# werner-duvaud/muzero-general

Hardware: AMD Instinct MI355X
Metric: mcts_simulations_per_sec (higher is better)
Workload: dtype f32; 1 GPU; C2 CartPole FullyConnectedNetwork, 4096 trees x 50 sims per GPU; trees_per_gpu=4096, num_simulations=50, action_space=2, network=fullyconnected, search_kernel=mzx::fc2_search_kernel, tree_statistics_dtype=f64, weights=reference constructor, torch.manual_seed(0) (RCCL-broadcast flat buffer)

## Files before the change

muzero-general_amd/csrc/mzx_fused_fc.h:

```cpp
#pragma once
#include <stdlib.h>

#include "mzx_search.h"

namespace mzx {

constexpr int FUSED_ROW = 16;
constexpr int FUSED_MAX_WIDTH = 64;
constexpr int FUSED_SCRATCH = 5 * FUSED_MAX_WIDTH;
constexpr int FUSED_PROF_WORDS = 16;

inline int row_action_lanes(const SearchParams& p) {
  const bool wide = p.num_actions > FUSED_ROW || 2 * p.support_size + 1 > 2 * FUSED_ROW;
  return wide ? 0 : (p.num_actions <= 4 ? 4 : 16);
}

struct FusedMlp {
  int32_t n;
  int32_t sizes[MZX_MAX_LAYERS + 2];
  int32_t w[MZX_MAX_LAYERS + 1], b[MZX_MAX_LAYERS + 1];
};

struct FusedFcArgs {
  SearchParams p;
// ... 277 lines not shown
      const int ld = (c == top) ? (depth & (FUSED_ROW - 1)) : FUSED_ROW - 1;
      const bool same = (k.tp == r.c.to_play);
      const double r_eff = (P == 1 || !same) ? k.rr : -k.rr;
      double my_in = val;
      chain_step<FUSED_ROW - 1>(r_eff, p.discount, ld, sub, val, my_in);
      if (sub == 0) my_in = val;
      if (c > 0) val = bcast_d<0>(r_eff) + p.discount * val;
      double qv = 0.0;
      if (k.active) {
        const double vs2 = k.vs + ((P == 1 || same) ? my_in : -my_in);
        const int vc2 = k.vc + 1;
        const double mean = vs2 / (double)vc2;
        qv = k.rr + p.discount * ((P == 1) ? mean : -mean);
        t.value_sum(k.n) = vs2;
        t.visit(k.n) = vc2;
        if (k.par >= 0) { t.slot_visit(k.par, k.ps) = vc2; t.slot_q(k.par, k.ps) = qv; }
        if (k.is_leaf) {
          t.child(k.par, k.ps) = k.n;
          t.parent(k.n) = k.par; t.parent_slot(k.n) = k.ps; t.to_play(k.n) = r.c.to_play; t.reward(k.n) = reward;
        }
      }
      const double h2 = row_max_d<16>(k.active ? qv : -MZX_INF), l2 = row_min_d16(k.active ? qv : MZX_INF);
      hi = h2 > hi ? h2 : hi;
      lo = l2 < lo ? l2 : lo;
      k = up;
    }
    if (hi > st.mx) st.mx = hi;
    if (lo < st.mn) st.mn = lo;
    return;
  }
  if (depth >= FUSED_ROW) {
    if (sub == 0) {
      store_state(t, st);
      t.child(r.c.parent, r.c.slot) = r.c.leaf;
      t.parent(r.c.leaf) = r.c.parent; t.parent_slot(r.c.leaf) = r.c.slot; t.to_play(r.c.leaf) = r.c.to_play;
      t.reward(r.c.leaf) = reward; t.visit(r.c.leaf) = 0; t.value_sum(r.c.leaf) = 0.0;
      tree_backprop(t, p, r.c, value);
    }
    wave_sync();
    st.mn = t.mm_min(); st.mx = t.mm_max();
    return;
  }
  const bool active = sub <= depth, is_leaf = sub == depth;
  const int n = r.my_node;
  double rr = reward, vs = 0.0;
  int vc = 0, tp = r.c.to_play;
  if (active && !is_leaf) {
    rr = t.reward(n); vs = t.value_sum(n); vc = t.visit(n);
    if (P == 2) tp = t.to_play(n);
  }
  const bool same = (tp == r.c.to_play);
  const double r_eff = (P == 1 || !same) ? rr : -rr;
  double val = value, my_in = value;
  chain_step<FUSED_ROW - 1>(r_eff, p.discount, depth, sub, val, my_in);
  if (sub == 0) my_in = val;
  double qv = 0.0;
  if (active) {
    const double vs2 = vs + ((P == 1 || same) ? my_in : -my_in);
    const int vc2 = vc + 1;
    const double mean = vs2 / (double)vc2;
    qv = rr + p.discount * ((P == 1) ? mean : -mean);
    t.value_sum(n) = vs2;
    t.visit(n) = vc2;
    if (sub > 0) { t.slot_visit(r.my_parent, r.my_pslot) = vc2; t.slot_q(r.my_parent, r.my_pslot) = qv; }
    if (is_leaf) {
      t.child(r.my_parent, r.my_pslot) = n;
      t.parent(n) = r.my_parent; t.parent_slot(n) = r.my_pslot; t.to_play(n) = r.c.to_play; t.reward(n) = reward;
    }
  }
  if (row_bits(__ballot(active && (qv > st.mx || qv < st.mn)), row_in_wave)) {
    const double hi = row_max_d<16>(active ? qv : -MZX_INF), lo = row_min_d16(active ? qv : MZX_INF);
    if (hi > st.mx) st.mx = hi;
    if (lo < st.mn) st.mn = lo;
  }
}


struct NetOut { float value, reward, policy; };

struct LdsNet {
  const float* W;
  const FusedFcArgs* a;

  __device__ __forceinline__ void stage_mlp(const FusedMlp& m, const float* flat, float* w, int tid) {
    for (int l = 0; l < m.n; ++l) {
      const int K = m.sizes[l], O = m.sizes[l + 1], base = m.w[l];
      for (int i = tid; i < O * K; i += blockDim.x) {
        const int o = i / K, k = i - o * K;
        w[base + k * O + o] = flat[base + i];
      }
      for (int i = tid; i < O; i += blockDim.x) w[m.b[l] + i] = flat[m.b[l] + i];
    }
  }
  __device__ __forceinline__ void stage(const FusedFcArgs& args, char* smem, int tid) {
    float* w = (float*)(smem + args.lds_weights);
    stage_mlp(args.rep, args.flat, w, tid);
    stage_mlp(args.dyn, args.flat, w, tid);
    stage_mlp(args.rew, args.flat, w, tid);
    stage_mlp(args.pol, args.flat, w, tid);
    stage_mlp(args.val, args.flat, w, tid);
  }
  __device__ __forceinline__ void setup(const FusedFcArgs& args, char* smem, int) {
    W = (const float*)(smem + args.lds_weights);
    a = &args;
  }

  template <int G>
  __device__ __forceinline__ void layer(const float* wl, const float* bl, const float* x, float* y, int K, int Kx, int O,
                                        int sub, int action, bool onehot, bool last) const {
    for (int o0 = sub; o0 < O; o0 += G * FUSED_ROW) {
      const float* wr = wl + o0;
      float acc[G];
#pragma unroll
      for (int j = 0; j < G; ++j) acc[j] = 0.f;
      int k = 0;
      constexpr int U = (G == 1) ? 8 : 4;
      for (; k + U <= Kx; k += U) {
        float xv[U], wv[U][G];
#pragma unroll
        for (int u = 0; u < U; ++u) {
          xv[u] = x[k + u];
#pragma unroll
          for (int j = 0; j < G; ++j) wv[u][j] = wr[(k + u) * O + j * FUSED_ROW];
        }
#pragma unroll
        for (int u = 0; u < U; ++u)
#pragma unroll
          for (int j = 0; j < G; ++j) acc[j] = fmaf(xv[u], wv[u][j], acc[j]);
      }
      for (; k < Kx; ++k) {
        const float xk = x[k];
#pragma unroll
        for (int j = 0; j < G; ++j) acc[j] = fmaf(xk, wr[k * O + j * FUSED_ROW], acc[j]);
      }
#pragma unroll
      for (int j = 0; j < G; ++j) {
        const int o = o0 + j * FUSED_ROW;
        if (o < O) {
          float v = acc[j];
          if (onehot) v += wr[(Kx + action) * O + j * FUSED_ROW];
          v += bl[o];
          y[o] = last ? v : mzx_elu(v);
        }
      }
    }
  }

  __device__ __forceinline__ void mlp(const FusedMlp& m, const float* x, float* tmp0, float* tmp1, float* out, int sub,
                                      int action, int onehot) const {
    for (int l = 0; l < m.n; ++l) {
      const int K = m.sizes[l], O = m.sizes[l + 1];
      const int Kx = (l == 0) ? K - onehot : K;
      const bool last = (l == m.n - 1);
      float* y = last ? out : ((l & 1) ? tmp1 : tmp0);
      const float* wl = W + m.w[l];
      const float* bl = W + m.b[l];
      const bool oh = (l == 0 && onehot);
      if (O > 2 * FUSED_ROW) layer<4>(wl, bl, x, y, K, Kx, O, sub, action, oh, last);
      else if (O > FUSED_ROW) layer<2>(wl, bl, x, y, K, Kx, O, sub, action, oh, last);
      else layer<1>(wl, bl, x, y, K, Kx, O, sub, action, oh, last);
      wave_sync();
      x = y;
    }
  }
  __device__ __forceinline__ void scale(const float* x, float* y, int E, int sub) const {
    float lo = x[0], hi = x[0];
    for (int k = 1; k < E; ++k) { lo = fminf(lo, x[k]); hi = fmaxf(hi, x[k]); }
    float sc = hi - lo;
    if (sc < 1e-5f) sc += 1e-5f;
    for (int j = sub; j < E; j += FUSED_ROW) y[j] = mzx_div(x[j] - lo, sc);
    wave_sync();
  }
  __device__ __forceinline__ float decode(const float* lg, int sub) const {
    const int F = 2 * a->p.support_size + 1, S = a->p.support_size;
    float m = -MZX_INF;
    for (int i = sub; i < F; i += FUSED_ROW) m = fmaxf(m, lg[i]);
    m = row_max(m);
    float den = 0.f;
    for (int i = sub; i < F; i += FUSED_ROW) den += mzx_expf(lg[i] - m);
    den = row_sum(den);
    float num = 0.f;
    for (int i = sub; i < F; i += FUSED_ROW) num += (float)(i - S) * mzx_div(mzx_expf(lg[i] - m), den);
    return support_inverse_transform(row_sum(num));
  }
  __device__ __forceinline__ void heads(const float* h, float* scr, int sub, NetOut& o) const {
    float* s0 = scr; float* s1 = scr + FUSED_MAX_WIDTH; float* s2 = scr + 2 * FUSED_MAX_WIDTH;
    float* s3 = scr + 3 * FUSED_MAX_WIDTH;
// ... 70 lines not shown

__device__ __forceinline__ void dot8x3_bcast(float xs, float xh, const float (&wr)[8], const float (&wp)[8],
                                             const float (&wv)[8], float& r, float& p, float& v) {
  float a = 0.f, b = 0.f, c = 0.f;
#define MZX_STEP3(K, J) MZX_FD_X("%[a]", "%[xs]", "%[r" #J "]", K) MZX_FD_X("%[b]", "%[xh]", "%[p" #J "]", K) MZX_FD_X("%[c]", "%[xh]", "%[v" #J "]", K)
  asm("s_nop 1\n\t" MZX_STEP3(0, 0) MZX_STEP3(1, 1) MZX_STEP3(2, 2) MZX_STEP3(3, 3)
      : [a] "+v"(a), [b] "+v"(b), [c] "+v"(c)
      : [xs] "v"(xs), [xh] "v"(xh), [r0] "v"(wr[0]), [r1] "v"(wr[1]), [r2] "v"(wr[2]), [r3] "v"(wr[3]),
        [p0] "v"(wp[0]), [p1] "v"(wp[1]), [p2] "v"(wp[2]), [p3] "v"(wp[3]),
        [v0] "v"(wv[0]), [v1] "v"(wv[1]), [v2] "v"(wv[2]), [v3] "v"(wv[3]));
  asm("s_nop 1\n\t" MZX_STEP3(4, 0) MZX_STEP3(5, 1) MZX_STEP3(6, 2) MZX_STEP3(7, 3)
      : [a] "+v"(a), [b] "+v"(b), [c] "+v"(c)
      : [xs] "v"(xs), [xh] "v"(xh), [r0] "v"(wr[4]), [r1] "v"(wr[5]), [r2] "v"(wr[6]), [r3] "v"(wr[7]),
        [p0] "v"(wp[4]), [p1] "v"(wp[5]), [p2] "v"(wp[6]), [p3] "v"(wp[7]),
        [v0] "v"(wv[4]), [v1] "v"(wv[5]), [v2] "v"(wv[6]), [v3] "v"(wv[7]));
#undef MZX_STEP3
  r = a; p = b; v = c;
}

__device__ __forceinline__ void dot16x5_bcast(float xr, float xp, float xv, const float (&ra)[16], const float (&rb)[16],
                                              const float (&pw)[16], const float (&va)[16], const float (&vb)[16],
                                              float& o_ra, float& o_rb, float& o_p, float& o_va, float& o_vb) {
  float a = 0.f, b = 0.f, c = 0.f, d = 0.f, e = 0.f;
#define MZX_STEP5(K, J)                                                                                             \
  MZX_FD_X("%[a]", "%[xr]", "%[s" #J "]", K) MZX_FD_X("%[b]", "%[xr]", "%[t" #J "]", K) MZX_FD_X("%[c]", "%[xp]", "%[u" #J "]", K) \
  MZX_FD_X("%[d]", "%[xv]", "%[w" #J "]", K) MZX_FD_X("%[e]", "%[xv]", "%[z" #J "]", K)
#define MZX_BLOCK5(K0, K1, K2, K3, B)                                                                              \
  asm("s_nop 1\n\t" MZX_STEP5(K0, 0) MZX_STEP5(K1, 1) MZX_STEP5(K2, 2) MZX_STEP5(K3, 3)                             \
      : [a] "+v"(a), [b] "+v"(b), [c] "+v"(c), [d] "+v"(d), [e] "+v"(e)                                             \
      : [xr] "v"(xr), [xp] "v"(xp), [xv] "v"(xv),                                                                    \
        [s0] "v"(ra[B]), [s1] "v"(ra[B + 1]), [s2] "v"(ra[B + 2]), [s3] "v"(ra[B + 3]),                               \
        [t0] "v"(rb[B]), [t1] "v"(rb[B + 1]), [t2] "v"(rb[B + 2]), [t3] "v"(rb[B + 3]),                               \
        [u0] "v"(pw[B]), [u1] "v"(pw[B + 1]), [u2] "v"(pw[B + 2]), [u3] "v"(pw[B + 3]),                               \
        [w0] "v"(va[B]), [w1] "v"(va[B + 1]), [w2] "v"(va[B + 2]), [w3] "v"(va[B + 3]),                               \
        [z0] "v"(vb[B]), [z1] "v"(vb[B + 1]), [z2] "v"(vb[B + 2]), [z3] "v"(vb[B + 3]))
  MZX_BLOCK5(0, 1, 2, 3, 0);
  MZX_BLOCK5(4, 5, 6, 7, 4);
  MZX_BLOCK5(8, 9, 10, 11, 8);
  MZX_BLOCK5(12, 13, 14, 15, 12);
#undef MZX_BLOCK5
#undef MZX_STEP5
  o_ra = a; o_rb = b; o_p = c; o_va = d; o_vb = e;
}

__device__ __forceinline__ void row_decode2x2(float a0, float a1, float b0, float b1, int F, int support, int sub,
                                              float& out_a, float& out_b) {
  const bool v0 = sub < F, v1 = sub + 16 < F;
  float ma = fmaxf(v0 ? a0 : -MZX_INF, v1 ? a1 : -MZX_INF), mb = fmaxf(v0 ? b0 : -MZX_INF, v1 ? b1 : -MZX_INF);
  row_max_2(ma, mb);
  const float ea0 = v0 ? mzx_expf(a0 - ma) : 0.f, ea1 = v1 ? mzx_expf(a1 - ma) : 0.f;
  const float eb0 = v0 ? mzx_expf(b0 - mb) : 0.f, eb1 = v1 ? mzx_expf(b1 - mb) : 0.f;
  float da = 0.f, db = 0.f;
  da += ea0; db += eb0;
  if (v1) { da += ea1; db += eb1; }
  const float dena = row_sum(da), denb = row_sum(db);
  float na = 0.f, nb = 0.f;
  if (v0) { na += (float)(sub - support) * mzx_div(ea0, dena); nb += (float)(sub - support) * mzx_div(eb0, denb); }
  if (v1) { na += (float)(sub + 16 - support) * mzx_div(ea1, dena); nb += (float)(sub + 16 - support) * mzx_div(eb1, denb); }
  support_inverse_transform_2(row_sum(na), row_sum(nb), sub, out_a, out_b);
}

template <int K, int I = 0>
__device__ __forceinline__ float fma_bcast(float x, const float (&w)[K], float acc) {
  if constexpr (I < K) {
    acc = fmaf(bcast<I>(x), w[I], acc);
    return fma_bcast<K, I + 1>(x, w, acc);
  } else {
    return acc;
  }
}
template <int K>
__device__ __forceinline__ float dot_bcast(float x, const float (&w)[K]) {
  if constexpr (K == 8) return dot8_bcast(x, w);
  else if constexpr (K == 16) return dot16_bcast(x, w);
  else return fma_bcast<K>(x, w, 0.f);
}
template <int K>
__device__ __forceinline__ void dot2_bcast(float x, const float (&u)[K], const float (&v)[K], float& ru, float& rv) {
  if constexpr (K == 16) dot16x2_bcast(x, u, v, ru, rv);
  else { ru = fma_bcast<K>(x, u, 0.f); rv = fma_bcast<K>(x, v, 0.f); }
}

template <int K>
__device__ __forceinline__ void load_row(float (&w)[K], float& b, const float* flat, int woff, int boff, int o, int O) {
  const bool ok = o < O;
#pragma unroll
  for (int k = 0; k < K; ++k) w[k] = ok ? flat[woff + o * K + k] : 0.f;
  b = ok ? flat[boff + o] : 0.f;
}

template <int IN, int E, int A, int F, int HD, int HR, int HP, int HV>
struct SmallNet {
  static_assert(IN <= 64 && E <= 16 && A <= 16 && F <= 32 && HD <= 16 && HR <= 16 && HP <= 16 && HV <= 16, "shape");
  float w_rep[IN], b_rep;
  float w_d1[E + A], b_d1, w_d2[HD], b_d2;
  float w_r1[E], b_r1, w_r2a[HR], b_r2a, w_r2b[HR], b_r2b;
  float w_p1[E], b_p1, w_p2[HP], b_p2;
  float w_v1[E], b_v1, w_v2a[HV], b_v2a, w_v2b[HV], b_v2b;
  int support;

  static bool matches(const FusedFcArgs& a) {
    const int Fa = 2 * a.p.support_size + 1;
    return a.in_size == IN && a.E == E && a.p.num_actions == A && Fa == F && a.rep.n == 1 && a.dyn.n == 2 &&
           a.dyn.sizes[1] == HD && a.rew.n == 2 && a.rew.sizes[1] == HR && a.pol.n == 2 && a.pol.sizes[1] == HP &&
           a.val.n == 2 && a.val.sizes[1] == HV;
  }

  __device__ __forceinline__ void stage(const FusedFcArgs&, char*, int) {}
  __device__ __forceinline__ void setup(const FusedFcArgs& a, char*, int sub) {
    const float* f = a.flat;
    support = a.p.support_size;
    load_row(w_rep, b_rep, f, a.rep.w[0], a.rep.b[0], sub, E);
    load_row(w_d1, b_d1, f, a.dyn.w[0], a.dyn.b[0], sub, HD);
    load_row(w_d2, b_d2, f, a.dyn.w[1], a.dyn.b[1], sub, E);
    load_row(w_r1, b_r1, f, a.rew.w[0], a.rew.b[0], sub, HR);
    load_row(w_r2a, b_r2a, f, a.rew.w[1], a.rew.b[1], sub, F);
    load_row(w_r2b, b_r2b, f, a.rew.w[1], a.rew.b[1], sub + 16, F);
    load_row(w_p1, b_p1, f, a.pol.w[0], a.pol.b[0], sub, HP);
    load_row(w_p2, b_p2, f, a.pol.w[1], a.pol.b[1], sub, A);
    load_row(w_v1, b_v1, f, a.val.w[0], a.val.b[0], sub, HV);
    load_row(w_v2a, b_v2a, f, a.val.w[1], a.val.b[1], sub, F);
    load_row(w_v2b, b_v2b, f, a.val.w[1], a.val.b[1], sub + 16, F);
  }

  __device__ __forceinline__ float scale(float s, int sub) const {
    const bool in = sub < E;
    float lo = in ? s : MZX_INF, hi = in ? s : -MZX_INF;
    row_min_max(lo, hi);
    float sc = hi - lo;
    if (sc < 1e-5f) sc += 1e-5f;
    return mzx_div(s - lo, sc);
  }
  __device__ __forceinline__ void heads(float hn, int sub, NetOut& o) const {
    const float p1 = mzx_elu(dot_bcast<E>(hn, w_p1) + b_p1);
    const float v1 = mzx_elu(dot_bcast<E>(hn, w_v1) + b_v1);
    o.policy = dot_bcast<HP>(p1, w_p2) + b_p2;
    float va, vb;
    dot2_bcast<HV>(v1, w_v2a, w_v2b, va, vb);
    o.value = row_decode2(va + b_v2a, vb + b_v2b, F, support, sub);
  }
  __device__ __forceinline__ void initial(const float* obs, float* h_out, float*, int sub, NetOut& o) const {
    float acc = 0.f;
#pragma unroll
    for (int k = 0; k < IN; ++k) acc = fmaf(obs[k], w_rep[k], acc);
    const float hn = scale(acc + b_rep, sub);
    h_out[sub] = hn;
    heads(hn, sub, o);
  }
  __device__ __forceinline__ void recurrent(const float* h_in, int action, float* h_out, float*, int sub,
                                            NetOut& o) const {
    float acc = 0.f;
#pragma unroll
    for (int k = 0; k < E; ++k) acc = fmaf(h_in[k], w_d1[k], acc);
    float col = w_d1[E];
#pragma unroll
    for (int x = 1; x < A; ++x) col = (action == x) ? w_d1[E + x] : col;
    const float d1 = mzx_elu((acc + col) + b_d1);
    const float s = dot_bcast<HD>(d1, w_d2) + b_d2;
    if constexpr (E == 8 && HR == 16 && HP == 16 && HV == 16) {
      const float hn = scale(s, sub);
      h_out[sub] = hn;
      float r1, p1, v1;
      dot8x3_bcast(s, hn, w_r1, w_p1, w_v1, r1, p1, v1);
      r1 = mzx_elu(r1 + b_r1); p1 = mzx_elu(p1 + b_p1); v1 = mzx_elu(v1 + b_v1);
      float ra, rb, pl, va, vb;
      dot16x5_bcast(r1, p1, v1, w_r2a, w_r2b, w_p2, w_v2a, w_v2b, ra, rb, pl, va, vb);
      o.policy = pl + b_p2;
      row_decode2x2(va + b_v2a, vb + b_v2b, ra + b_r2a, rb + b_r2b, F, support, sub, o.value, o.reward);
      return;
    }
    const float r1 = mzx_elu(dot_bcast<E>(s, w_r1) + b_r1);
    float ra, rb;
    dot2_bcast<HR>(r1, w_r2a, w_r2b, ra, rb);
    const float hn = scale(s, sub);
    h_out[sub] = hn;
    o.reward = row_decode2(ra + b_r2a, rb + b_r2b, F, support, sub);
    heads(hn, sub, o);
  }
};


#define MZX_PROF(k)                                             \
  if (PROFILE) {                                                \
    __builtin_amdgcn_sched_barrier(0);                          \
    asm volatile("s_waitcnt vmcnt(0) lgkmcnt(0)" ::: "memory"); \
    const unsigned long long _t = __builtin_readcyclecounter(); \
    prof[k] += (uint32_t)(_t - t_last);                         \
    t_last = _t;                                                \
    __builtin_amdgcn_sched_barrier(0);                          \
  }

template <class Net, int AW, bool PROFILE>
__global__ void __launch_bounds__(256) fused_fc_search_kernel(const FusedFcArgs a) {
  extern __shared__ __attribute__((aligned(16))) char smem[];
  const int tid = threadIdx.x;
  const int sub = tid & (FUSED_ROW - 1);
  const int row = tid / FUSED_ROW;
  const int row_in_wave = row & 3;
  const int tree = blockIdx.x * a.trees_per_block + row;
  const int A = a.p.num_actions, E = a.E;
  uint32_t prof[FUSED_PROF_WORDS];
  unsigned long long t_last = 0;
  if (PROFILE) {
    for (int k = 0; k < FUSED_PROF_WORDS; ++k) prof[k] = 0;
    t_last = __builtin_readcyclecounter();
  }

  Net net;
  double* tables = (double*)(smem + a.lds_tables);
  const int ntab = 2 * (a.p.num_nodes + 1);
  for (int i = tid; i < ntab; i += blockDim.x) tables[i] = a.tables[i];
  net.stage(a, smem, tid);
  __syncthreads();
  if (row >= a.trees_per_block || tree >= a.p.num_trees) return;
  net.setup(a, smem, sub);

  char* slab = smem + a.lds_trees + (size_t)row * a.tree_stride;
  TreeRef t;
  t.base = slab;
  t.L = a.L;
  float* hidden = (float*)(slab + a.off_hidden);
  float* scr = (float*)(slab + a.off_scratch);

  SearchParams p = a.p;
  p.pbc_table = tables;
  p.sqrt_table = tables + (a.p.num_nodes + 1);
  const uint32_t* tape = (const uint32_t*)a.io.d_tape + (size_t)tree * p.tape_words;
// ... 210 lines not shown
```

muzero-general_amd/csrc/mzx_fused_fc2.h:

```cpp
#pragma once
#include "mzx_fused_fc.h"

namespace mzx {

struct Fc2Args {
  const float* ov_hidden;
  const double* ov_priors;
  const double* ov_reward;
  FusedFcArgs f;
  int32_t off_slots, off_nodes, off_path, off_roota, off_mm, off_hidden, off_scratch;
  int32_t tree_stride, lds_inv;
};

#ifndef MZX_HOSTCHECK

struct __attribute__((aligned(16))) Fc2Slot {
  double ps;
  double q;
  int32_t n;
  int32_t child;
  double prior;
};
struct __attribute__((aligned(16))) Fc2Node {
  double value_sum, reward;
// ... 1 lines not shown
};
static_assert(sizeof(Fc2Slot) == 32 && sizeof(Fc2Node) == 32, "record size");

__device__ __forceinline__ double recip_refined(double b) {
  const double y0 = __builtin_amdgcn_rcp(b);
  const double f0 = __builtin_fma(-b, y0, 1.0);
  const double f1 = __builtin_fma(y0, f0, y0);
  const double f2 = __builtin_fma(-b, f1, 1.0);
  return __builtin_fma(f1, f2, f1);
}
__device__ __forceinline__ double div_by(double a, double b, double y) {
  const double m = a * y;
  const double r = __builtin_fma(-b, m, a);
  const double q = __builtin_fma(r, y, m);
  return __builtin_amdgcn_div_fixup(q, b, a);
}
__device__ __forceinline__ double prior_score(double pbcN, double sqN, int n, double inv_n1, double prior) {
  const double pb_c = pbcN * div_by(sqN, (double)(n + 1), inv_n1);
  return pb_c * prior;
}

template <int W>
__device__ __forceinline__ float row_sum_w(float v) {
  v = v + dpp_f<DPP_XOR1>(v);
  if constexpr (W > 2) v = v + dpp_f<DPP_XOR2>(v);
  if constexpr (W > 4) v = v + dpp_f<DPP_HALF_MIRROR>(v);
  if constexpr (W > 8) v = v + dpp_f<DPP_MIRROR>(v);
  return v;
}
constexpr int DPP_ROW_SHL1 = 0x101;
__device__ __forceinline__ int shl1_i(int v, int old) {
  return __builtin_amdgcn_update_dpp(old, v, DPP_ROW_SHL1, 0xF, 0xF, false);
}
__device__ __forceinline__ double shl1_d(double v, double old) {
  return __hiloint2double(shl1_i(__double2hiint(v), __double2hiint(old)), shl1_i(__double2loint(v), __double2loint(old)));
}

template <int J>
__device__ __forceinline__ void chain_step2(double r_eff, double disc, unsigned lim, int sub, double& val) {
  const bool on = (unsigned)(J - 1 - sub) < lim;
  __builtin_amdgcn_sched_barrier(0);
  const double rj = bcast_d<J>(r_eff);
  const double nv = rj + disc * val;
  val = on ? nv : val;
}
__device__ __forceinline__ void value_chain(double r_eff, double disc, int ld, int sub, int wmax, double& val) {
  const int room = ld - sub;
  const unsigned lim = (unsigned)(room > 0 ? room : 0);
  if (wmax >= 13) {
    chain_step2<15>(r_eff, disc, lim, sub, val);
    chain_step2<14>(r_eff, disc, lim, sub, val);
    chain_step2<13>(r_eff, disc, lim, sub, val);
  }
  if (wmax >= 9) {
    chain_step2<12>(r_eff, disc, lim, sub, val);
    chain_step2<11>(r_eff, disc, lim, sub, val);
    chain_step2<10>(r_eff, disc, lim, sub, val);
    chain_step2<9>(r_eff, disc, lim, sub, val);
  }
  if (wmax >= 7) {
    chain_step2<8>(r_eff, disc, lim, sub, val);
    chain_step2<7>(r_eff, disc, lim, sub, val);
  }
  chain_step2<6>(r_eff, disc, lim, sub, val);
  chain_step2<5>(r_eff, disc, lim, sub, val);
  chain_step2<4>(r_eff, disc, lim, sub, val);
  chain_step2<3>(r_eff, disc, lim, sub, val);
  chain_step2<2>(r_eff, disc, lim, sub, val);
  chain_step2<1>(r_eff, disc, lim, sub, val);
}



struct Fc2Tree {
  Fc2Slot* slots;
  Fc2Node* nodes;
  int2* path;
  int32_t* roota;
  double* mm;
  const double *pbc, *sqt, *inv_y;
  double pb_leaf, disc;
  int A, NN, P;
};
struct Fc2Row { int32_t n_nodes, tape_pos, flags, ties, max_depth, sum_depth, root_n, root_to_play; };
struct Fc2Walk { int parent, slot, leaf, depth, levels, vtp, action; };

template <int AW>
__device__ __forceinline__ Fc2Walk fc2_walk(const Fc2Tree& T, Fc2Row& st, const uint32_t* tape, int tape_words, int sub,
                                            int row_in_wave) {
  const double2 mmv = *(const double2*)T.mm;
  const double mn = mmv.x, mx = mmv.y;
  const double dd = mx - mn;
  const double yd = recip_refined(dd);
  const bool norm_on = mx > mn;
  int node = 0, depth = 0, slot = 0;
  int levels = 0;
  if constexpr (AW == 2) {
    const double mn_e = norm_on ? mn : 0.0, dd_e = norm_on ? dd : 1.0, yd_e = norm_on ? yd : 1.0;
    unsigned long long more = __builtin_amdgcn_ballot_w64(true);
    do {
      const bool act = __builtin_amdgcn_inverse_ballot_w64(more);
      ++levels;
      asm volatile("" : "+s"(levels));
      const Fc2Slot* rp = T.slots + (node * 2 + (sub & 1));
      const double ps = rp->ps, q = rp->q;
      const int n = rp->n, c = rp->child;
      const bool seen = n > 0;
      __builtin_amdgcn_sched_barrier(0);
      const double v = div_by(q - mn_e, dd_e, yd_e);
      const double wv = ps + v;
      const double sc = seen ? wv : ps;
      const double a0 = bcast_d<0>(sc), a1 = bcast_d<1>(sc);
      const int c0 = bcast_i<0>(c), c1 = bcast_i<1>(c);
      const bool up = a1 > a0;
      int sl = up ? 1 : 0;
      int cw = up ? c1 : c0;
      const bool eq = a0 == a1;
      if (__builtin_expect((__builtin_amdgcn_ballot_w64(eq) & more) != 0, 0)) {
        if (eq && act) {
          ++st.ties;
          sl = tape_draw(tape, tape_words, st.tape_pos, st.flags, 2);
          cw = sl ? c1 : c0;
        }
      }
      cw = act ? cw : -1;
      T.path[depth + 1] = make_int2(cw, sl);
      depth += act ? 1 : 0;
      asm volatile("" : "+v"(depth));
      slot = act ? sl : slot;
      const bool go = cw >= 0;
      node = go ? cw : node;
      more = __builtin_amdgcn_ballot_w64(go);
    } while (more != 0);
  } else {
  bool done = false;
  for (;;) {
    ++levels;
    const Fc2Slot* rp = T.slots + (node * AW + (sub & (AW - 1)));
    const double ps = rp->ps, q = rp->q;
    const int n = rp->n, c = rp->child;
    const double nv = div_by(q - mn, dd, yd);
    const double v = norm_on ? nv : q;
    const double wv = ps + v;
    const double sc = (n > 0) ? wv : ps;
    int sl, cw;
    {
      const double best = row_max_d<AW>(sc);
      const unsigned bits = row_bits(__ballot(sc == best), row_in_wave) & ((1u << AW) - 1u);
      const int nbest = __popc(bits);
      sl = nbest ? (__ffs(bits) - 1) : 0;
      if (__builtin_expect(nbest > 1 && !done, 0)) {
        ++st.ties;
        int k = tape_draw(tape, tape_words, st.tape_pos, st.flags, nbest);
        unsigned b = bits;
        for (; k > 0; --k) b &= b - 1;
        sl = __ffs(b) - 1;
      }
      if constexpr (AW <= 4) cw = pick_i<AW>(c, sl);
      else cw = perm_i(c, sl, row_in_wave);
    }
    const bool act = !done;
    cw = act ? cw : -1;
    T.path[depth + 1] = make_int2(cw, sl);
    depth += act ? 1 : 0;
    slot = act ? sl : slot;
    const bool go = cw >= 0;
    node = go ? cw : node;
    done = !go;
    if (__builtin_amdgcn_ballot_w64(go) == 0) break;
  }
  }
  Fc2Walk w;
  w.vtp = (T.P == 1) ? 0 : ((st.root_to_play + depth) & 1);
  int leaf = st.n_nodes;
  if (leaf >= T.NN) { st.flags |= TF_NODE_OVERFLOW; leaf = T.NN - 1; }
  T.path[depth] = make_int2(leaf, slot);
  const int ra = T.roota[slot < AW ? slot : 0];
  w.parent = node; w.slot = slot; w.leaf = leaf; w.depth = depth; w.levels = levels;
  w.action = (node == 0) ? ra : slot;
  return w;
}

template <int AW>
struct Fc2Lane {
  int nd, pslot, par, vc, tp, rpar;
  double vs, rr, inv_vc2, inv_vc3, pb, sv;
  int sn[AW <= 4 ? AW : 1];
  double sprior[AW <= 4 ? AW : 1], sinv[AW <= 4 ? AW : 1];
};

template <int AW>
__device__ __forceinline__ Fc2Lane<AW> fc2_load_lane(const Fc2Tree& T, const Fc2Walk& w, int c, int sub) {
  Fc2Lane<AW> L;
  const int d = c * 16 + sub;
  const bool inner = d < w.depth;
  const int dq = inner ? d : w.depth;
  const int2 pe = T.path[dq];
  L.nd = pe.x; L.pslot = pe.y;
  L.par = T.path[dq > 0 ? dq - 1 : 0].x;
  const int nr = inner ? L.nd : L.par;
  const Fc2Node* np = T.nodes + nr;
  const double vs = np->value_sum;
  const int4 hv = *(const int4*)&np->visit;
  L.rr = np->reward;
  L.vs = inner ? vs : 0.0; L.vc = inner ? hv.x : 0;
  L.tp = inner ? hv.y : w.vtp;
  L.rpar = inner ? hv.z : L.par;
  L.inv_vc2 = T.inv_y[L.vc + 1];
  L.inv_vc3 = T.inv_y[L.vc + 2];
  L.pb = T.pbc[L.vc + 1]; L.sv = T.sqt[L.vc + 1];
  if constexpr (AW <= 4) {
#pragma unroll
    for (int s = 0; s < AW; ++s) { L.sn[s] = T.slots[nr * AW + s].n; L.sprior[s] = T.slots[nr * AW + s].prior; }
#pragma unroll
    for (int s = 0; s < AW; ++s) L.sinv[s] = T.inv_y[L.sn[s] + 1];
  }
  return L;
}

template <int AW>
__device__ __forceinline__ void fc2_expand(const Fc2Tree& T, int leaf, int sub, bool in, double prior) {
  Fc2Slot s;
  s.prior = in ? prior : 0.0;
  s.q = 0.0; s.n = 0; s.child = -1;
  s.ps = in ? T.pb_leaf * s.prior : -MZX_INF;
  static_assert(AW <= 4 || AW == FUSED_ROW, "a dead slot row exists for 2- and 4-lane records only");
  int at = leaf * AW + sub;
  if constexpr (AW < FUSED_ROW) at = (sub < AW) ? at : -AW;
  T.slots[at] = s;
}

template <int AW>
__device__ __forceinline__ void fc2_backprop(const Fc2Tree& T, Fc2Row& st, const Fc2Walk& w, Fc2Lane<AW> L, int sub,
                                             double value, double reward) {
  static_assert(AW <= 4 || AW == FUSED_ROW, "a dead slot row exists for 2- and 4-lane records only");
  const int depth = w.depth, vtp = w.vtp, P = T.P;
// ... 29 lines not shown
      r.value_sum = vs2; r.reward = rr; r.visit = vc2; r.to_play = L.tp; r.parent = L.rpar; r.parent_slot = L.pslot;
      T.nodes[L.nd] = r;
      if (AW <= 4 || d > 0) {
        Fc2Slot* ps = T.slots + (L.par * AW + L.pslot);
        ps->q = qv;
        *(int2*)&ps->n = make_int2(vc2, L.nd);
      }
      if (d <= depth) {
        __hip_atomic_fetch_min(&T.mm[0], qv, __ATOMIC_RELAXED, __HIP_MEMORY_SCOPE_WORKGROUP);
        __hip_atomic_fetch_max(&T.mm[1], qv, __ATOMIC_RELAXED, __HIP_MEMORY_SCOPE_WORKGROUP);
      }
    }
    if constexpr (AW <= 4) {
      const int ch_vc2 = shl1_i(vc2, carry_vc2), ch_slot = shl1_i(L.pslot, carry_pslot);
      const double ch_inv = shl1_d(L.inv_vc3, carry_inv);
      const int nslots = (L.nd == 0) ? st.root_n : T.A;
      Fc2Slot* sp = T.slots + (inner ? L.nd : -1) * AW;
#pragma unroll
      for (int s = 0; s < AW; ++s) {
        const bool on_path = (s == ch_slot);
        const int ns = on_path ? ch_vc2 : L.sn[s];
        const double iv = on_path ? ch_inv : L.sinv[s];
        const double psc = prior_score(L.pb, L.sv, ns, iv, L.sprior[s]);
        sp[s].ps = (s < nslots) ? psc : -MZX_INF;
      }
      carry_vc2 = bcast_i<0>(vc2); carry_pslot = bcast_i<0>(L.pslot); carry_inv = bcast_d<0>(L.inv_vc3);
    } else {
      wave_sync();
      if (inner) {
        Fc2Slot* sp = T.slots + L.nd * AW;
        const int nslots = (L.nd == 0) ? st.root_n : T.A;
        for (int s = 0; s < nslots; ++s) {
          const int ns = sp[s].n;
          sp[s].ps = prior_score(L.pb, L.sv, ns, T.inv_y[ns + 1], sp[s].prior);
        }
      }
    }
  }
  wave_sync();
}

template <int RW>
__device__ __forceinline__ void fc2_from_arena(const Fc2Tree& FT, Fc2Row& rst, const TreeRef& t, int sub) {
  const int nn = t.meta(TM_N_NODES), rootn = t.meta(TM_ROOT_N);
  for (int n = sub; n < nn; n += FUSED_ROW) {
    Fc2Node r;
    r.value_sum = t.value_sum(n); r.reward = t.reward(n); r.visit = t.visit(n); r.to_play = t.to_play(n);
    r.parent = t.parent(n); r.parent_slot = t.parent_slot(n);
    FT.nodes[n] = r;
    const int nc = (n == 0) ? rootn : FT.A;
    for (int s2 = 0; s2 < RW; ++s2) {
      Fc2Slot q;
      const bool in = s2 < nc;
      q.prior = in ? t.prior(n, s2) : 0.0; q.q = in ? t.slot_q(n, s2) : 0.0;
      q.n = in ? t.slot_visit(n, s2) : 0; q.child = in ? t.child(n, s2) : -1;
      q.ps = in ? prior_score(FT.pbc[r.visit], FT.sqt[r.visit], q.n, FT.inv_y[q.n + 1], q.prior) : -MZX_INF;
      FT.slots[n * RW + s2] = q;
    }
  }
  if (sub < RW) FT.roota[sub] = (sub < rootn) ? t.root_action(sub) : -1;
  if (sub == 0) { FT.path[0] = make_int2(0, -1); FT.mm[0] = t.mm_min(); FT.mm[1] = t.mm_max(); }
  rst.n_nodes = nn; rst.tape_pos = t.meta(TM_TAPE_POS); rst.flags = t.meta(TM_FLAGS); rst.ties = t.meta(TM_TIE_DRAWS);
  rst.max_depth = t.meta(TM_MAX_DEPTH); rst.sum_depth = t.meta(TM_SUM_DEPTH); rst.root_n = rootn;
  rst.root_to_play = t.to_play(0);
}

template <class Net, int AW, bool PROFILE, bool CONT = false>
__global__ void __launch_bounds__(256) fc2_search_kernel(const Fc2Args a) {
  extern __shared__ __attribute__((aligned(16))) char smem[];
  const int tid = threadIdx.x;
  const int sub = tid & (FUSED_ROW - 1);
  const int row = tid / FUSED_ROW;
  const int row_in_wave = row & 3;
  const int tree = blockIdx.x * a.f.trees_per_block + row;
  const int A = a.f.p.num_actions, E = a.f.E, NN = a.f.p.num_nodes, P = a.f.p.num_players;
  const double disc = a.f.p.discount;
  uint32_t prof[FUSED_PROF_WORDS];
  unsigned long long t_last = 0;
  if (PROFILE) {
    for (int k = 0; k < FUSED_PROF_WORDS; ++k) prof[k] = 0;
    t_last = __builtin_readcyclecounter();
  }

  Net net;
  double* tables = (double*)(smem + a.f.lds_tables);
  double* inv_y = (double*)(smem + a.lds_inv);
  const int ntab = 2 * (NN + 1);
  for (int i = tid; i < ntab; i += blockDim.x) tables[i] = a.f.tables[i];
  for (int i = tid; i < NN + 2; i += blockDim.x) inv_y[i] = recip_refined((double)(i > 0 ? i : 1));
  net.stage(a.f, smem, tid);
  __syncthreads();
  if (row >= a.f.trees_per_block || tree >= a.f.p.num_trees) return;
  net.setup(a.f, smem, sub);
  const double* pbc = tables;
  const double* sqt = tables + (NN + 1);
  const double pb_leaf = pbc[1] * div_by(sqt[1], 1.0, inv_y[1]);

  char* slab = smem + a.f.lds_trees + (size_t)row * a.tree_stride;
  Fc2Slot* slots = (Fc2Slot*)(slab + a.off_slots);
  Fc2Node* nodes = (Fc2Node*)(slab + a.off_nodes);
  int2* path = (int2*)(slab + a.off_path);
  int32_t* roota = (int32_t*)(slab + a.off_roota);
  double* mm = (double*)(slab + a.off_mm);
  float* hidden = (float*)(slab + a.off_hidden);
  float* scr = (float*)(slab + a.off_scratch);
  const uint32_t* tape = (const uint32_t*)a.f.io.d_tape + (size_t)tree * a.f.p.tape_words;
  const int tape_words = a.f.p.tape_words;

  int32_t n_nodes = 1, tape_pos = 0, flags = 0, ties = 0, max_depth = 0, sum_depth = 0, root_n = 0, root_to_play = 0;
  MZX_PROF(0)

  if constexpr (CONT) {
    Fc2Tree FT;
    FT.slots = slots; FT.nodes = nodes; FT.path = path; FT.roota = roota; FT.mm = mm;
    FT.pbc = pbc; FT.sqt = sqt; FT.inv_y = inv_y; FT.A = A;
    TreeRef t;
    t.base = a.f.export_trees + (size_t)tree * a.f.L.tree_bytes;
    t.L = a.f.L;
    Fc2Row rst;
    fc2_from_arena<AW>(FT, rst, t, sub);
    n_nodes = rst.n_nodes; tape_pos = rst.tape_pos; flags = rst.flags; ties = rst.ties; max_depth = rst.max_depth;
    sum_depth = rst.sum_depth; root_n = rst.root_n; root_to_play = rst.root_to_play;
    const float* hd = a.f.export_hidden + (size_t)tree * NN * E;
    for (int i = sub; i < n_nodes * E; i += FUSED_ROW) hidden[i] = hd[i];
    wave_sync();
  }
  if constexpr (!CONT) {
    NetOut o;
    const bool given = a.ov_hidden != nullptr;
    if (!given) net.initial(a.f.io.d_observation + (size_t)tree * a.f.in_size, hidden, scr, sub, o);
    else
      for (int e = sub; e < E; e += FUSED_ROW) hidden[e] = a.ov_hidden[(size_t)tree * E + e];
    const int32_t* lg = a.f.io.d_legal_actions + (size_t)tree * A;
    const double* nz = a.f.io.d_noise ? a.f.io.d_noise + (size_t)tree * A : nullptr;
    while (root_n < A && lg[root_n] >= 0) ++root_n;
    if (!given && sub < A) scr[sub] = o.policy;
    wave_sync();
    const bool in = sub < root_n;
    const float l = (in && !given) ? scr[lg[sub]] : -MZX_INF;
    const float m = row_max_w<AW>(l);
    const float e = (in && !given) ? mzx_expf(l - m) : 0.f;
    const float den = row_sum_w<AW>(e);
    root_to_play = a.f.io.d_to_play[tree];
    if (sub == 0) {
      Fc2Node r;
      r.value_sum = 0.0; r.visit = 0; r.to_play = root_to_play;
      r.reward = given ? a.ov_reward[tree] : (double)support_inverse_transform(0.0f);
      r.parent = -1; r.parent_slot = -1;
      nodes[0] = r;
      path[0] = make_int2(0, -1);
      mm[0] = MZX_INF; mm[1] = -MZX_INF;
      if (!given && a.f.io.d_root_predicted_value) a.f.io.d_root_predicted_value[tree] = (double)o.value;
    }
    if (sub < AW) {
      Fc2Slot s;
      const double pr = !in ? 0.0 : (given ? a.ov_priors[(size_t)tree * A + sub] : (double)mzx_div(e, den));
      s.prior = in ? root_noisy_prior(pr, nz, sub, a.f.p.exploration_fraction) : 0.0;
      s.q = 0.0; s.n = 0; s.child = -1;
      s.ps = in ? prior_score(pbc[0], sqt[0], 0, inv_y[1], s.prior) : -MZX_INF;
      slots[sub] = s;
      roota[sub] = in ? lg[sub] : -1;
    }
    wave_sync();
  }
  MZX_PROF(1)

  Fc2Tree T;
  T.slots = slots; T.nodes = nodes; T.path = path; T.roota = roota; T.mm = mm;
  T.pbc = pbc; T.sqt = sqt; T.inv_y = inv_y; T.pb_leaf = pb_leaf; T.disc = disc; T.A = A; T.NN = NN; T.P = P;
  Fc2Row st;
  st.n_nodes = n_nodes; st.tape_pos = tape_pos; st.flags = flags; st.ties = ties; st.max_depth = max_depth;
  st.sum_depth = sum_depth; st.root_n = root_n; st.root_to_play = root_to_play;
  const int num_sims = a.f.p.num_sims;
  for (int sim = 0; sim < num_sims; ++sim) {
    const Fc2Walk w = fc2_walk<AW>(T, st, tape, tape_words, sub, row_in_wave);
    MZX_PROF(2)
    wave_sync();
    const Fc2Lane<AW> L = fc2_load_lane<AW>(T, w, w.levels >> 4, sub);
    MZX_PROF(7)

    NetOut o;
    net.recurrent(hidden + w.parent * E, w.action, hidden + w.leaf * E, scr, sub, o);
    MZX_PROF(3)

    {
      const bool in = sub < A;
      const float m = row_max_w<AW>(in ? o.policy : -MZX_INF);
      const float e = in ? mzx_expf(o.policy - m) : 0.f;
      const float den = row_sum_w<AW>(e);
      fc2_expand<AW>(T, w.leaf, sub, in, (double)mzx_div(e, den));
    }
    MZX_PROF(4)

    fc2_backprop<AW>(T, st, w, L, sub, (double)o.value, (double)o.reward);
    MZX_PROF(5)
  }
  n_nodes = st.n_nodes; tape_pos = st.tape_pos; flags = st.flags; ties = st.ties; max_depth = st.max_depth;
  sum_depth = st.sum_depth;

  if (sub == 0) {
    for (int x = 0; x < A; ++x) a.f.io.d_visit_counts[(size_t)tree * A + x] = 0;
    for (int s = 0; s < root_n; ++s) a.f.io.d_visit_counts[(size_t)tree * A + roota[s]] = slots[s].n;
    const int vc = nodes[0].visit;
    a.f.io.d_root_value[tree] = (vc == 0) ? 0.0 : nodes[0].value_sum / (double)vc;
    a.f.io.d_info[tree * 4 + 0] = max_depth;
    a.f.io.d_info[tree * 4 + 1] = flags;
    a.f.io.d_info[tree * 4 + 2] = tape_pos;
    a.f.io.d_info[tree * 4 + 3] = sum_depth;
  }
  if (a.f.export_trees) {
    TreeRef t;
    t.base = a.f.export_trees + (size_t)tree * a.f.L.tree_bytes;
    t.L = a.f.L;
    for (int n = sub; n < n_nodes; n += FUSED_ROW) {
      const Fc2Node r = nodes[n];
      t.value_sum(n) = r.value_sum; t.reward(n) = r.reward; t.visit(n) = r.visit; t.to_play(n) = r.to_play;
      t.parent(n) = r.parent; t.parent_slot(n) = r.parent_slot;
      for (int s = 0; s < A; ++s) {
        const Fc2Slot q = slots[n * AW + s];
        t.prior(n, s) = q.prior; t.slot_q(n, s) = q.q; t.slot_visit(n, s) = q.n; t.child(n, s) = q.child;
      }
    }
    if (sub == 0) {
      for (int k = 0; k < TM_WORDS; ++k) t.meta(k) = 0;
      t.mm_min() = mm[0]; t.mm_max() = mm[1];
      t.meta(TM_N_NODES) = n_nodes; t.meta(TM_TAPE_POS) = tape_pos; t.meta(TM_FLAGS) = flags;
      t.meta(TM_TIE_DRAWS) = ties; t.meta(TM_MAX_DEPTH) = max_depth; t.meta(TM_SUM_DEPTH) = sum_depth;
      t.meta(TM_ROOT_N) = root_n;
      for (int s = 0; s < A; ++s) t.root_action(s) = roota[s];
    }
    float* hd = a.f.export_hidden + (size_t)tree * NN * E;
    for (int i = sub; i < n_nodes * E; i += FUSED_ROW) hd[i] = hidden[i];
  }
  MZX_PROF(6)
  if (PROFILE && sub == 0 && a.f.prof)
    for (int k = 0; k < FUSED_PROF_WORDS; ++k) a.f.prof[(size_t)tree * FUSED_PROF_WORDS + k] = prof[k];
}


struct Fc2Plan {
  Fc2Args args;
  int lds_bytes = 0, ok = 0, small = 0, aw = 0;
};

inline Fc2Plan fc2_plan(const mzx_search* s, bool allow_small = true) {
  Fc2Plan P;
  const FusedPlan base = fused_plan(s, allow_small);
  if (!base.ok) return P;
  Fc2Args& a = P.args;
  memset(&a, 0, sizeof(a));
  a.f = base.args;
  P.small = base.small;
  const int A = s->p.num_actions, N = s->p.num_nodes, E = a.f.E;
  const int AW = A <= 2 ? 2 : (A <= 4 ? 4 : 16);
  P.aw = AW;
  auto al16 = [](int64_t x) { return (x + 15) & ~int64_t(15); };
  int64_t o = 0;
  a.f.lds_tables = (int32_t)o;  o += al16(int64_t(16) * (N + 1));
// ... 80 lines not shown
```

Measured before the change: 1.425 billion sims/s.

## Hoist all per-tree global loads before barrier to overlap kernel prologue latency

The prologue now issues every global read up front, before the block barrier: register weight rows, the observation vector, legal actions, noise, to_play, the first tape word and override inputs. Zero-masking and the use of these values are deferred until afterwards, so their latency overlaps the LDS table staging and the barrier instead of being serialized. LDS weight staging is batched into groups of loads followed by transposed stores, and the root legal-action count is computed with a ballot rather than a serial loop. The first tie-break tape draw reuses the prefetched word. Registers go up (x_obs, ov_h, prefetch temporaries), and the first-draw logic has to reproduce tape_draw exactly.

After: 1.408 billion sims/s. -1.2%, worse.

```diff
diff --git a/muzero-general_amd/csrc/mzx_fused_fc.h b/muzero-general_amd/csrc/mzx_fused_fc.h
--- a/muzero-general_amd/csrc/mzx_fused_fc.h
+++ b/muzero-general_amd/csrc/mzx_fused_fc.h
@@ -383,14 +383,36 @@
   const float* W;
   const FusedFcArgs* a;
 
+  static constexpr int STAGE_BATCH = 8;
+  __device__ __forceinline__ void stage_words(const float* src, float* dst, int n, int K, int O, int tid) {
+    const int bd = (int)blockDim.x;
+    const int dq = bd / K, dr = bd - dq * K;
+    for (int i0 = tid; i0 < n; i0 += STAGE_BATCH * bd) {
+      float v[STAGE_BATCH];
+#pragma unroll
+      for (int j = 0; j < STAGE_BATCH; ++j) {
+        const int i = i0 + j * bd;
+        v[j] = src[i < n ? i : n - 1];
+      }
+      int o = i0 / K, k = i0 - o * K;
+#pragma unroll
+      for (int j = 0; j < STAGE_BATCH; ++j) {
+        const int i = i0 + j * bd;
+        if (i < n) dst[k * O + o] = v[j];
+        o += dq; k += dr;
+        if (k >= K) { k -= K; ++o; }
+      }
+    }
+  }
   __device__ __forceinline__ void stage_mlp(const FusedMlp& m, const float* flat, float* w, int tid) {
     for (int l = 0; l < m.n; ++l) {
-      const int K = m.sizes[l], O = m.sizes[l + 1], base = m.w[l];
-      for (int i = tid; i < O * K; i += blockDim.x) {
-        const int o = i / K, k = i - o * K;
-        w[base + k * O + o] = flat[base + i];
-      }
-      for (int i = tid; i < O; i += blockDim.x) w[m.b[l] + i] = flat[m.b[l] + i];
+      const int K = m.sizes[l], O = m.sizes[l + 1];
+      const float* fb = flat + m.b[l];
+      float* wb = w + m.b[l];
+      const float bv = fb[tid < O ? tid : O - 1];
+      stage_words(flat + m.w[l], w + m.w[l], O * K, K, O, tid);
+      if (tid < O) wb[tid] = bv;
+      for (int i = tid + (int)blockDim.x; i < O; i += blockDim.x) wb[i] = fb[i];
     }
   }
   __device__ __forceinline__ void stage(const FusedFcArgs& args, char* smem, int tid) {
@@ -404,6 +426,11 @@
   __device__ __forceinline__ void setup(const FusedFcArgs& args, char* smem, int) {
     W = (const float*)(smem + args.lds_weights);
     a = &args;
+  }
+  __device__ __forceinline__ void request(const FusedFcArgs&, const float*, int) {}
+  __device__ __forceinline__ void finish(const FusedFcArgs& args, char* smem, int sub) { setup(args, smem, sub); }
+  __device__ __forceinline__ void initial_requested(const float* obs, float* h_out, float* scr, int sub, NetOut& o) const {
+    initial(obs, h_out, scr, sub, o);
   }
 
   template <int G>
@@ -640,11 +667,23 @@
 }
 
 template <int K>
+__device__ __forceinline__ void request_row(float (&w)[K], float& b, const float* flat, int woff, int boff, int o, int O) {
+  const int oc = o < O ? o : O - 1;
+#pragma unroll
+  for (int k = 0; k < K; ++k) w[k] = flat[woff + oc * K + k];
+  b = flat[boff + oc];
+}
+template <int K>
+__device__ __forceinline__ void zero_row(float (&w)[K], float& b, int o, int O) {
+  const bool ok = o < O;
+#pragma unroll
+  for (int k = 0; k < K; ++k) w[k] = ok ? w[k] : 0.f;
+  b = ok ? b : 0.f;
+}
+template <int K>
 __device__ __forceinline__ void load_row(float (&w)[K], float& b, const float* flat, int woff, int boff, int o, int O) {
-  const bool ok = o < O;
-#pragma unroll
-  for (int k = 0; k < K; ++k) w[k] = ok ? flat[woff + o * K + k] : 0.f;
-  b = ok ? flat[boff + o] : 0.f;
+  request_row(w, b, flat, woff, boff, o, O);
+  zero_row(w, b, o, O);
 }
 
 template <int IN, int E, int A, int F, int HD, int HR, int HP, int HV>
@@ -655,6 +694,7 @@
   float w_r1[E], b_r1, w_r2a[HR], b_r2a, w_r2b[HR], b_r2b;
   float w_p1[E], b_p1, w_p2[HP], b_p2;
   float w_v1[E], b_v1, w_v2a[HV], b_v2a, w_v2b[HV], b_v2b;
+  float x_obs[IN];
   int support;
 
   static bool matches(const FusedFcArgs& a) {
@@ -665,20 +705,39 @@
   }
 
   __device__ __forceinline__ void stage(const FusedFcArgs&, char*, int) {}
-  __device__ __forceinline__ void setup(const FusedFcArgs& a, char*, int sub) {
+  __device__ __forceinline__ void request(const FusedFcArgs& a, const float* obs, int sub) {
     const float* f = a.flat;
     support = a.p.support_size;
-    load_row(w_rep, b_rep, f, a.rep.w[0], a.rep.b[0], sub, E);
-    load_row(w_d1, b_d1, f, a.dyn.w[0], a.dyn.b[0], sub, HD);
-    load_row(w_d2, b_d2, f, a.dyn.w[1], a.dyn.b[1], sub, E);
-    load_row(w_r1, b_r1, f, a.rew.w[0], a.rew.b[0], sub, HR);
-    load_row(w_r2a, b_r2a, f, a.rew.w[1], a.rew.b[1], sub, F);
-    load_row(w_r2b, b_r2b, f, a.rew.w[1], a.rew.b[1], sub + 16, F);
-    load_row(w_p1, b_p1, f, a.pol.w[0], a.pol.b[0], sub, HP);
-    load_row(w_p2, b_p2, f, a.pol.w[1], a.pol.b[1], sub, A);
-    load_row(w_v1, b_v1, f, a.val.w[0], a.val.b[0], sub, HV);
-    load_row(w_v2a, b_v2a, f, a.val.w[1], a.val.b[1], sub, F);
-    load_row(w_v2b, b_v2b, f, a.val.w[1], a.val.b[1], sub + 16, F);
+#pragma unroll
+    for (int k = 0; k < IN; ++k) x_obs[k] = obs[k];
+    request_row(w_rep, b_rep, f, a.rep.w[0], a.rep.b[0], sub, E);
+    request_row(w_d1, b_d1, f, a.dyn.w[0], a.dyn.b[0], sub, HD);
+    request_row(w_d2, b_d2, f, a.dyn.w[1], a.dyn.b[1], sub, E);
+    request_row(w_r1, b_r1, f, a.rew.w[0], a.rew.b[0], sub, HR);
+    request_row(w_r2a, b_r2a, f, a.rew.w[1], a.rew.b[1], sub, F);
+    request_row(w_r2b, b_r2b, f, a.rew.w[1], a.rew.b[1], sub + 16, F);
+    request_row(w_p1, b_p1, f, a.pol.w[0], a.pol.b[0], sub, HP);
+    request_row(w_p2, b_p2, f, a.pol.w[1], a.pol.b[1], sub, A);
+    request_row(w_v1, b_v1, f, a.val.w[0], a.val.b[0], sub, HV);
+    request_row(w_v2a, b_v2a, f, a.val.w[1], a.val.b[1], sub, F);
+    request_row(w_v2b, b_v2b, f, a.val.w[1], a.val.b[1], sub + 16, F);
+  }
+  __device__ __forceinline__ void finish(const FusedFcArgs&, char*, int sub) {
+    zero_row(w_rep, b_rep, sub, E);
+    zero_row(w_d1, b_d1, sub, HD);
+    zero_row(w_d2, b_d2, sub, E);
+    zero_row(w_r1, b_r1, sub, HR);
+    zero_row(w_r2a, b_r2a, sub, F);
+    zero_row(w_r2b, b_r2b, sub + 16, F);
+    zero_row(w_p1, b_p1, sub, HP);
+    zero_row(w_p2, b_p2, sub, A);
+    zero_row(w_v1, b_v1, sub, HV);
+    zero_row(w_v2a, b_v2a, sub, F);
+    zero_row(w_v2b, b_v2b, sub + 16, F);
+  }
+  __device__ __forceinline__ void setup(const FusedFcArgs& a, char* smem, int sub) {
+    request(a, a.flat, sub);
+    finish(a, smem, sub);
   }
 
   __device__ __forceinline__ float scale(float s, int sub) const {
@@ -701,6 +760,14 @@
     float acc = 0.f;
 #pragma unroll
     for (int k = 0; k < IN; ++k) acc = fmaf(obs[k], w_rep[k], acc);
+    const float hn = scale(acc + b_rep, sub);
+    h_out[sub] = hn;
+    heads(hn, sub, o);
+  }
+  __device__ __forceinline__ void initial_requested(const float*, float* h_out, float*, int sub, NetOut& o) const {
+    float acc = 0.f;
+#pragma unroll
+    for (int k = 0; k < IN; ++k) acc = fmaf(x_obs[k], w_rep[k], acc);
     const float hn = scale(acc + b_rep, sub);
     h_out[sub] = hn;
     heads(hn, sub, o);
diff --git a/muzero-general_amd/csrc/mzx_fused_fc2.h b/muzero-general_amd/csrc/mzx_fused_fc2.h
--- a/muzero-general_amd/csrc/mzx_fused_fc2.h
+++ b/muzero-general_amd/csrc/mzx_fused_fc2.h
@@ -107,12 +107,24 @@
   double pb_leaf, disc;
   int A, NN, P;
 };
+__device__ __forceinline__ int tape_draw_first(const uint32_t* tape, int tape_words, int32_t& pos, int32_t& flags, int n,
+                                               uint32_t w0, bool first) {
+  if (first) {
+    uint32_t rng = (uint32_t)(n - 1), mask = rng;
+    mask |= mask >> 1; mask |= mask >> 2; mask |= mask >> 4; mask |= mask >> 8; mask |= mask >> 16;
+    pos = 1;
+    const uint32_t w = w0 & mask;
+    if (w <= rng) return (int)w;
+  }
+  return tape_draw(tape, tape_words, pos, flags, n);
+}
+
 struct Fc2Row { int32_t n_nodes, tape_pos, flags, ties, max_depth, sum_depth, root_n, root_to_play; };
 struct Fc2Walk { int parent, slot, leaf, depth, levels, vtp, action; };
 
 template <int AW>
 __device__ __forceinline__ Fc2Walk fc2_walk(const Fc2Tree& T, Fc2Row& st, const uint32_t* tape, int tape_words, int sub,
-                                            int row_in_wave) {
+                                            int row_in_wave, uint32_t w0 = 0, bool w0_first = false) {
   const double2 mmv = *(const double2*)T.mm;
   const double mn = mmv.x, mx = mmv.y;
   const double dd = mx - mn;
@@ -144,7 +156,7 @@
       if (__builtin_expect((__builtin_amdgcn_ballot_w64(eq) & more) != 0, 0)) {
         if (eq && act) {
           ++st.ties;
-          sl = tape_draw(tape, tape_words, st.tape_pos, st.flags, 2);
+          sl = tape_draw_first(tape, tape_words, st.tape_pos, st.flags, 2, w0, w0_first);
           cw = sl ? c1 : c0;
         }
       }
@@ -176,7 +188,7 @@
       sl = nbest ? (__ffs(bits) - 1) : 0;
       if (__builtin_expect(nbest > 1 && !done, 0)) {
         ++st.ties;
-        int k = tape_draw(tape, tape_words, st.tape_pos, st.flags, nbest);
+        int k = tape_draw_first(tape, tape_words, st.tape_pos, st.flags, nbest, w0, w0_first);
         unsigned b = bits;
         for (; k > 0; --k) b &= b - 1;
         sl = __ffs(b) - 1;
@@ -372,16 +384,46 @@
     t_last = __builtin_readcyclecounter();
   }
 
+  const bool live = row < a.f.trees_per_block && tree < a.f.p.num_trees;
+  const int tq = live ? tree : 0;
+  const int sa = sub < A ? sub : A - 1;
+  const int tape_words = a.f.p.tape_words;
+  const bool given = !CONT && a.ov_hidden != nullptr;
+  const bool noisy = a.f.io.d_noise != nullptr;
+  const bool w0_pre = !CONT && tape_words > 0;
   Net net;
   double* tables = (double*)(smem + a.f.lds_tables);
   double* inv_y = (double*)(smem + a.lds_inv);
   const int ntab = 2 * (NN + 1);
-  for (int i = tid; i < ntab; i += blockDim.x) tables[i] = a.f.tables[i];
+  const double tab0 = a.f.tables[tid < ntab ? tid : ntab - 1];
+  net.request(a.f, (CONT || given) ? a.f.flat : a.f.io.d_observation + (size_t)tq * a.f.in_size, sub);
+  int32_t lg_mine = -1, tp_pre = 0;
+  uint32_t w0 = 0;
+  double nz_mine = 0.0, ov_prior = 0.0, ov_rew = 0.0;
+  float ov_h[FUSED_MAX_WIDTH / FUSED_ROW] = {};
+  if constexpr (!CONT) {
+    lg_mine = a.f.io.d_legal_actions[(size_t)tq * A + sa];
+    nz_mine = *(noisy ? a.f.io.d_noise + (size_t)tq * A + sa : a.f.tables);
+    tp_pre = a.f.io.d_to_play[tq];
+    w0 = *(w0_pre ? (const uint32_t*)a.f.io.d_tape + (size_t)tq * tape_words : (const uint32_t*)a.f.tables);
+    if (given) {
+#pragma unroll
+      for (int j = 0; j < FUSED_MAX_WIDTH / FUSED_ROW; ++j) {
+        const int e = sub + j * FUSED_ROW;
+        ov_h[j] = a.ov_hidden[(size_t)tq * E + (e < E ? e : E - 1)];
+      }
+      ov_prior = a.ov_priors[(size_t)tq * A + sa];
+      ov_rew = a.ov_reward[tq];
+    }
+  }
+
   for (int i = tid; i < NN + 2; i += blockDim.x) inv_y[i] = recip_refined((double)(i > 0 ? i : 1));
+  if (tid < ntab) tables[tid] = tab0;
+  for (int i = tid + blockDim.x; i < ntab; i += blockDim.x) tables[i] = a.f.tables[i];
   net.stage(a.f, smem, tid);
   __syncthreads();
-  if (row >= a.f.trees_per_block || tree >= a.f.p.num_trees) return;
-  net.setup(a.f, smem, sub);
+  if (!live) return;
+  net.finish(a.f, smem, sub);
   const double* pbc = tables;
   const double* sqt = tables + (NN + 1);
   const double pb_leaf = pbc[1] * div_by(sqt[1], 1.0, inv_y[1]);
@@ -394,8 +436,7 @@
   double* mm = (double*)(slab + a.off_mm);
   float* hidden = (float*)(slab + a.off_hidden);
   float* scr = (float*)(slab + a.off_scratch);
-  const uint32_t* tape = (const uint32_t*)a.f.io.d_tape + (size_t)tree * a.f.p.tape_words;
-  const int tape_words = a.f.p.tape_words;
+  const uint32_t* tape = (const uint32_t*)a.f.io.d_tape + (size_t)tree * tape_words;
 
   int32_t n_nodes = 1, tape_pos = 0, flags = 0, ties = 0, max_depth = 0, sum_depth = 0, root_n = 0, root_to_play = 0;
   MZX_PROF(0)
@@ -417,25 +458,28 @@
   }
   if constexpr (!CONT) {
     NetOut o;
-    const bool given = a.ov_hidden != nullptr;
-    if (!given) net.initial(a.f.io.d_observation + (size_t)tree * a.f.in_size, hidden, scr, sub, o);
-    else
-      for (int e = sub; e < E; e += FUSED_ROW) hidden[e] = a.ov_hidden[(size_t)tree * E + e];
-    const int32_t* lg = a.f.io.d_legal_actions + (size_t)tree * A;
-    const double* nz = a.f.io.d_noise ? a.f.io.d_noise + (size_t)tree * A : nullptr;
-    while (root_n < A && lg[root_n] >= 0) ++root_n;
+    if (!given) net.initial_requested(a.f.io.d_observation + (size_t)tree * a.f.in_size, hidden, scr, sub, o);
+    else {
+#pragma unroll
+      for (int j = 0; j < FUSED_MAX_WIDTH / FUSED_ROW; ++j)
+        if (sub + j * FUSED_ROW < E) hidden[sub + j * FUSED_ROW] = ov_h[j];
+    }
+    {
+      const unsigned neg = row_bits(__builtin_amdgcn_ballot_w64(sub >= A || lg_mine < 0), row_in_wave);
+      root_n = neg ? __ffs(neg) - 1 : A;
+    }
     if (!given && sub < A) scr[sub] = o.policy;
     wave_sync();
     const bool in = sub < root_n;
-    const float l = (in && !given) ? scr[lg[sub]] : -MZX_INF;
+    const float l = (in && !given) ? scr[lg_mine] : -MZX_INF;
     const float m = row_max_w<AW>(l);
     const float e = (in && !given) ? mzx_expf(l - m) : 0.f;
     const float den = row_sum_w<AW>(e);
-    root_to_play = a.f.io.d_to_play[tree];
+    root_to_play = tp_pre;
     if (sub == 0) {
       Fc2Node r;
       r.value_sum = 0.0; r.visit = 0; r.to_play = root_to_play;
-      r.reward = given ? a.ov_reward[tree] : (double)support_inverse_transform(0.0f);
+      r.reward = given ? ov_rew : (double)support_inverse_transform(0.0f);
       r.parent = -1; r.parent_slot = -1;
       nodes[0] = r;
       path[0] = make_int2(0, -1);
@@ -444,12 +488,13 @@
     }
     if (sub < AW) {
       Fc2Slot s;
-      const double pr = !in ? 0.0 : (given ? a.ov_priors[(size_t)tree * A + sub] : (double)mzx_div(e, den));
-      s.prior = in ? root_noisy_prior(pr, nz, sub, a.f.p.exploration_fraction) : 0.0;
+      const double pr = !in ? 0.0 : (given ? ov_prior : (double)mzx_div(e, den));
+      const double frac = a.f.p.exploration_fraction;
+      s.prior = !in ? 0.0 : (noisy ? pr * (1.0 - frac) + nz_mine * frac : pr);
       s.q = 0.0; s.n = 0; s.child = -1;
       s.ps = in ? prior_score(pbc[0], sqt[0], 0, inv_y[1], s.prior) : -MZX_INF;
       slots[sub] = s;
-      roota[sub] = in ? lg[sub] : -1;
+      roota[sub] = in ? lg_mine : -1;
     }
     wave_sync();
   }
@@ -463,7 +508,7 @@
   st.sum_depth = sum_depth; st.root_n = root_n; st.root_to_play = root_to_play;
   const int num_sims = a.f.p.num_sims;
   for (int sim = 0; sim < num_sims; ++sim) {
-    const Fc2Walk w = fc2_walk<AW>(T, st, tape, tape_words, sub, row_in_wave);
+    const Fc2Walk w = fc2_walk<AW>(T, st, tape, tape_words, sub, row_in_wave, w0, w0_pre && sim == 0);
     MZX_PROF(2)
     wave_sync();
     const Fc2Lane<AW> L = fc2_load_lane<AW>(T, w, w.levels >> 4, sub);
```
